# cts198859/deeprl_network

Measured on NVIDIA H100. Metric: agent-env-steps/sec CACC Catch-up NeurComm A2C, higher is better.
Workload: dtype f32

## Files before the change

### deeprl_network_b200/csrc/tc.cuh

```cuda
#pragma once
#include <cuda_runtime.h>
#include <stdint.h>

namespace tc {

__device__ __forceinline__ uint32_t tf32_rn(float x) {
  uint32_t r;
  asm("cvt.rna.tf32.f32 %0, %1;" : "=r"(r) : "f"(x));
  return r;
}
__device__ __forceinline__ void split_tf32(float x, uint32_t& hi, uint32_t& lo) {
  hi = tf32_rn(x);
  lo = tf32_rn(x - __uint_as_float(hi));
}
__device__ __forceinline__ void split_tf32(float x, float& hi, float& lo) {
  uint32_t h, l;
  split_tf32(x, h, l);
  hi = __uint_as_float(h); lo = __uint_as_float(l);
}
__device__ __forceinline__ uint32_t smem_u32(const void* p) { return (uint32_t)__cvta_generic_to_shared(p); }

__device__ __forceinline__ void pdl_wait() { asm volatile("griddepcontrol.wait;" ::: "memory"); }
__device__ __forceinline__ void pdl_launch_dependents() { asm volatile("griddepcontrol.launch_dependents;" ::: "memory"); }

// ... 40 lines not shown
  return false;
}

__device__ __forceinline__ void bulk_g2s(void* smem_dst, const void* gsrc, uint32_t bytes, uint64_t* bar) {
  asm volatile("cp.async.bulk.shared::cluster.global.mbarrier::complete_tx::bytes [%0], [%1], %2, [%3];" ::"r"(
                   smem_u32(smem_dst)),
               "l"(gsrc), "r"(bytes), "r"(smem_u32(bar))
               : "memory");
}

__host__ __device__ inline uint32_t sw128_offset(uint32_t row, uint32_t k) {
  return (row >> 3) * 1024u + (row & 7u) * 128u + ((((k >> 2) ^ row) & 7u) << 4) + ((k & 3u) << 2);
}
__device__ __forceinline__ uint64_t smem_desc_sw128(const void* tile) {
  const uint64_t addr = (uint64_t)(smem_u32(tile) >> 4) & 0x3FFFull;
  return addr | (1ull << 16) | ((uint64_t)(1024 >> 4) << 32) | (1ull << 62);
}
__device__ __forceinline__ void st_hilo8(uint8_t* tile_hi, uint8_t* tile_lo, uint32_t row, uint32_t k0, const float (&x)[8]) {
  float h[8], l[8];
#pragma unroll
  for (int i = 0; i < 8; ++i) split_tf32(x[i], h[i], l[i]);
#pragma unroll
  for (int c = 0; c < 2; ++c) {
    const uint32_t off = sw128_offset(row, k0 + 4 * c);
    *reinterpret_cast<float4*>(tile_hi + off) = make_float4(h[4 * c], h[4 * c + 1], h[4 * c + 2], h[4 * c + 3]);
    *reinterpret_cast<float4*>(tile_lo + off) = make_float4(l[4 * c], l[4 * c + 1], l[4 * c + 2], l[4 * c + 3]);
  }
}
__device__ __forceinline__ void fence_proxy_async() { asm volatile("fence.proxy.async.shared::cta;" ::: "memory"); }

__device__ __forceinline__ void wgmma_fence() { asm volatile("wgmma.fence.sync.aligned;" ::: "memory"); }
__device__ __forceinline__ void wgmma_commit() { asm volatile("wgmma.commit_group.sync.aligned;" ::: "memory"); }
__device__ __forceinline__ void wgmma_wait_all() { asm volatile("wgmma.wait_group.sync.aligned 0;" ::: "memory"); }

__device__ __forceinline__ void wgmma_tf32_n64(float* d, uint64_t da, uint64_t db, uint32_t acc) {
  asm volatile(
      "{\n\t.reg .pred p;\n\tsetp.ne.b32 p, %34, 0;\n\t"
      "wgmma.mma_async.sync.aligned.m64n64k8.f32.tf32.tf32 {%0,%1,%2,%3,%4,%5,%6,%7,%8,%9,%10,%11,%12,%13,%14,%15,%16,%17,%18,%19,%20,%21,%22,%23,%24,%25,%26,%27,%28,%29,%30,%31}, %32, %33, p, 1, 1;\n\t}"
      : "+f"(d[0]), "+f"(d[1]), "+f"(d[2]), "+f"(d[3]), "+f"(d[4]), "+f"(d[5]), "+f"(d[6]), "+f"(d[7]), "+f"(d[8]), "+f"(d[9]), "+f"(d[10]), "+f"(d[11]), "+f"(d[12]), "+f"(d[13]), "+f"(d[14]), "+f"(d[15]), "+f"(d[16]), "+f"(d[17]), "+f"(d[18]), "+f"(d[19]), "+f"(d[20]), "+f"(d[21]), "+f"(d[22]), "+f"(d[23]), "+f"(d[24]), "+f"(d[25]), "+f"(d[26]), "+f"(d[27]), "+f"(d[28]), "+f"(d[29]), "+f"(d[30]), "+f"(d[31])
      : "l"(da), "l"(db), "r"(acc));
}
__device__ __forceinline__ void wgmma_tf32_n128(float* d, uint64_t da, uint64_t db, uint32_t acc) {
  asm volatile(
      "{\n\t.reg .pred p;\n\tsetp.ne.b32 p, %66, 0;\n\t"
      "wgmma.mma_async.sync.aligned.m64n128k8.f32.tf32.tf32 {%0,%1,%2,%3,%4,%5,%6,%7,%8,%9,%10,%11,%12,%13,%14,%15,%16,%17,%18,%19,%20,%21,%22,%23,%24,%25,%26,%27,%28,%29,%30,%31,%32,%33,%34,%35,%36,%37,%38,%39,%40,%41,%42,%43,%44,%45,%46,%47,%48,%49,%50,%51,%52,%53,%54,%55,%56,%57,%58,%59,%60,%61,%62,%63}, %64, %65, p, 1, 1;\n\t}"
      : "+f"(d[0]), "+f"(d[1]), "+f"(d[2]), "+f"(d[3]), "+f"(d[4]), "+f"(d[5]), "+f"(d[6]), "+f"(d[7]), "+f"(d[8]), "+f"(d[9]), "+f"(d[10]), "+f"(d[11]), "+f"(d[12]), "+f"(d[13]), "+f"(d[14]), "+f"(d[15]), "+f"(d[16]), "+f"(d[17]), "+f"(d[18]), "+f"(d[19]), "+f"(d[20]), "+f"(d[21]), "+f"(d[22]), "+f"(d[23]), "+f"(d[24]), "+f"(d[25]), "+f"(d[26]), "+f"(d[27]), "+f"(d[28]), "+f"(d[29]), "+f"(d[30]), "+f"(d[31]), "+f"(d[32]), "+f"(d[33]), "+f"(d[34]), "+f"(d[35]), "+f"(d[36]), "+f"(d[37]), "+f"(d[38]), "+f"(d[39]), "+f"(d[40]), "+f"(d[41]), "+f"(d[42]), "+f"(d[43]), "+f"(d[44]), "+f"(d[45]), "+f"(d[46]), "+f"(d[47]), "+f"(d[48]), "+f"(d[49]), "+f"(d[50]), "+f"(d[51]), "+f"(d[52]), "+f"(d[53]), "+f"(d[54]), "+f"(d[55]), "+f"(d[56]), "+f"(d[57]), "+f"(d[58]), "+f"(d[59]), "+f"(d[60]), "+f"(d[61]), "+f"(d[62]), "+f"(d[63])
      : "l"(da), "l"(db), "r"(acc));
}
__device__ __forceinline__ void wgmma_tf32_n192(float* d, uint64_t da, uint64_t db, uint32_t acc) {
  asm volatile(
      "{\n\t.reg .pred p;\n\tsetp.ne.b32 p, %98, 0;\n\t"
      "wgmma.mma_async.sync.aligned.m64n192k8.f32.tf32.tf32 {%0,%1,%2,%3,%4,%5,%6,%7,%8,%9,%10,%11,%12,%13,%14,%15,%16,%17,%18,%19,%20,%21,%22,%23,%24,%25,%26,%27,%28,%29,%30,%31,%32,%33,%34,%35,%36,%37,%38,%39,%40,%41,%42,%43,%44,%45,%46,%47,%48,%49,%50,%51,%52,%53,%54,%55,%56,%57,%58,%59,%60,%61,%62,%63,%64,%65,%66,%67,%68,%69,%70,%71,%72,%73,%74,%75,%76,%77,%78,%79,%80,%81,%82,%83,%84,%85,%86,%87,%88,%89,%90,%91,%92,%93,%94,%95}, %96, %97, p, 1, 1;\n\t}"
      : "+f"(d[0]), "+f"(d[1]), "+f"(d[2]), "+f"(d[3]), "+f"(d[4]), "+f"(d[5]), "+f"(d[6]), "+f"(d[7]), "+f"(d[8]), "+f"(d[9]), "+f"(d[10]), "+f"(d[11]), "+f"(d[12]), "+f"(d[13]), "+f"(d[14]), "+f"(d[15]), "+f"(d[16]), "+f"(d[17]), "+f"(d[18]), "+f"(d[19]), "+f"(d[20]), "+f"(d[21]), "+f"(d[22]), "+f"(d[23]), "+f"(d[24]), "+f"(d[25]), "+f"(d[26]), "+f"(d[27]), "+f"(d[28]), "+f"(d[29]), "+f"(d[30]), "+f"(d[31]), "+f"(d[32]), "+f"(d[33]), "+f"(d[34]), "+f"(d[35]), "+f"(d[36]), "+f"(d[37]), "+f"(d[38]), "+f"(d[39]), "+f"(d[40]), "+f"(d[41]), "+f"(d[42]), "+f"(d[43]), "+f"(d[44]), "+f"(d[45]), "+f"(d[46]), "+f"(d[47]), "+f"(d[48]), "+f"(d[49]), "+f"(d[50]), "+f"(d[51]), "+f"(d[52]), "+f"(d[53]), "+f"(d[54]), "+f"(d[55]), "+f"(d[56]), "+f"(d[57]), "+f"(d[58]), "+f"(d[59]), "+f"(d[60]), "+f"(d[61]), "+f"(d[62]), "+f"(d[63]), "+f"(d[64]), "+f"(d[65]), "+f"(d[66]), "+f"(d[67]), "+f"(d[68]), "+f"(d[69]), "+f"(d[70]), "+f"(d[71]), "+f"(d[72]), "+f"(d[73]), "+f"(d[74]), "+f"(d[75]), "+f"(d[76]), "+f"(d[77]), "+f"(d[78]), "+f"(d[79]), "+f"(d[80]), "+f"(d[81]), "+f"(d[82]), "+f"(d[83]), "+f"(d[84]), "+f"(d[85]), "+f"(d[86]), "+f"(d[87]), "+f"(d[88]), "+f"(d[89]), "+f"(d[90]), "+f"(d[91]), "+f"(d[92]), "+f"(d[93]), "+f"(d[94]), "+f"(d[95])
      : "l"(da), "l"(db), "r"(acc));
}
__device__ __forceinline__ void wgmma_tf32_n256(float* d, uint64_t da, uint64_t db, uint32_t acc) {
  asm volatile(
      "{\n\t.reg .pred p;\n\tsetp.ne.b32 p, %130, 0;\n\t"
      "wgmma.mma_async.sync.aligned.m64n256k8.f32.tf32.tf32 {%0,%1,%2,%3,%4,%5,%6,%7,%8,%9,%10,%11,%12,%13,%14,%15,%16,%17,%18,%19,%20,%21,%22,%23,%24,%25,%26,%27,%28,%29,%30,%31,%32,%33,%34,%35,%36,%37,%38,%39,%40,%41,%42,%43,%44,%45,%46,%47,%48,%49,%50,%51,%52,%53,%54,%55,%56,%57,%58,%59,%60,%61,%62,%63,%64,%65,%66,%67,%68,%69,%70,%71,%72,%73,%74,%75,%76,%77,%78,%79,%80,%81,%82,%83,%84,%85,%86,%87,%88,%89,%90,%91,%92,%93,%94,%95,%96,%97,%98,%99,%100,%101,%102,%103,%104,%105,%106,%107,%108,%109,%110,%111,%112,%113,%114,%115,%116,%117,%118,%119,%120,%121,%122,%123,%124,%125,%126,%127}, %128, %129, p, 1, 1;\n\t}"
      : "+f"(d[0]), "+f"(d[1]), "+f"(d[2]), "+f"(d[3]), "+f"(d[4]), "+f"(d[5]), "+f"(d[6]), "+f"(d[7]), "+f"(d[8]), "+f"(d[9]), "+f"(d[10]), "+f"(d[11]), "+f"(d[12]), "+f"(d[13]), "+f"(d[14]), "+f"(d[15]), "+f"(d[16]), "+f"(d[17]), "+f"(d[18]), "+f"(d[19]), "+f"(d[20]), "+f"(d[21]), "+f"(d[22]), "+f"(d[23]), "+f"(d[24]), "+f"(d[25]), "+f"(d[26]), "+f"(d[27]), "+f"(d[28]), "+f"(d[29]), "+f"(d[30]), "+f"(d[31]), "+f"(d[32]), "+f"(d[33]), "+f"(d[34]), "+f"(d[35]), "+f"(d[36]), "+f"(d[37]), "+f"(d[38]), "+f"(d[39]), "+f"(d[40]), "+f"(d[41]), "+f"(d[42]), "+f"(d[43]), "+f"(d[44]), "+f"(d[45]), "+f"(d[46]), "+f"(d[47]), "+f"(d[48]), "+f"(d[49]), "+f"(d[50]), "+f"(d[51]), "+f"(d[52]), "+f"(d[53]), "+f"(d[54]), "+f"(d[55]), "+f"(d[56]), "+f"(d[57]), "+f"(d[58]), "+f"(d[59]), "+f"(d[60]), "+f"(d[61]), "+f"(d[62]), "+f"(d[63]), "+f"(d[64]), "+f"(d[65]), "+f"(d[66]), "+f"(d[67]), "+f"(d[68]), "+f"(d[69]), "+f"(d[70]), "+f"(d[71]), "+f"(d[72]), "+f"(d[73]), "+f"(d[74]), "+f"(d[75]), "+f"(d[76]), "+f"(d[77]), "+f"(d[78]), "+f"(d[79]), "+f"(d[80]), "+f"(d[81]), "+f"(d[82]), "+f"(d[83]), "+f"(d[84]), "+f"(d[85]), "+f"(d[86]), "+f"(d[87]), "+f"(d[88]), "+f"(d[89]), "+f"(d[90]), "+f"(d[91]), "+f"(d[92]), "+f"(d[93]), "+f"(d[94]), "+f"(d[95]), "+f"(d[96]), "+f"(d[97]), "+f"(d[98]), "+f"(d[99]), "+f"(d[100]), "+f"(d[101]), "+f"(d[102]), "+f"(d[103]), "+f"(d[104]), "+f"(d[105]), "+f"(d[106]), "+f"(d[107]), "+f"(d[108]), "+f"(d[109]), "+f"(d[110]), "+f"(d[111]), "+f"(d[112]), "+f"(d[113]), "+f"(d[114]), "+f"(d[115]), "+f"(d[116]), "+f"(d[117]), "+f"(d[118]), "+f"(d[119]), "+f"(d[120]), "+f"(d[121]), "+f"(d[122]), "+f"(d[123]), "+f"(d[124]), "+f"(d[125]), "+f"(d[126]), "+f"(d[127])
      : "l"(da), "l"(db), "r"(acc));
}
__device__ __forceinline__ void wgmma_tf32(int N, float* d, uint64_t da, uint64_t db, uint32_t acc) {
  switch (N) {
    case 64: wgmma_tf32_n64(d, da, db, acc); break;
    case 128: wgmma_tf32_n128(d, da, db, acc); break;
    case 192: wgmma_tf32_n192(d, da, db, acc); break;
    default: wgmma_tf32_n256(d, da, db, acc); break;
  }
}
__device__ __forceinline__ void wgmma_kblock_3x(int N, float* d, uint64_t a_hi, uint64_t a_lo, uint64_t b_hi, uint64_t b_lo,
                                                int ksteps, bool first) {
  for (int ks = 0; ks < ksteps; ++ks) {
    wgmma_tf32(N, d, a_hi + 2 * ks, b_hi + 2 * ks, (first && ks == 0) ? 0u : 1u);
    wgmma_tf32(N, d, a_hi + 2 * ks, b_lo + 2 * ks, 1u);
    wgmma_tf32(N, d, a_lo + 2 * ks, b_hi + 2 * ks, 1u);
  }
}

}
```

### deeprl_network_b200/csrc/tc_bwd.cu

```cuda
#include "bwd_common.cuh"
#include "tc_row.cuh"

namespace {
using namespace tcrow;

template <int VAR, bool FM, bool RAW, int HW>
__global__ void __launch_bounds__(TC_THREADS, 1) tc_cell_bwd_kernel(const __grid_constant__ nmarl_model m,
                                                                    const __grid_constant__ BwdK k) {
  extern __shared__ uint8_t smem_raw[];
  const Smem sm = smem_map(smem_raw);
  KbEnt* sched = sm.sched;

  const int i = blockIdx.y;
  const nmarl_agent& ag = m.agent[i];
  const int B = k.B, b0 = blockIdx.x * ROWS;
  const int tid = threadIdx.x, warp = tid >> 5, lane = tid & 31;
  const int n_a = m.n_a, SD = m.s_dim;
  const float* __restrict__ P = k.params;
  constexpr int NGRP = (VAR == NMARL_NC) ? 4 : 2;
  const int Km = (VAR == NMARL_IC3) ? NH : ag.n_nbr * NH;

  if (tid == 0) {
    init_barriers(sm);
    int n = 0;
    const int korder[8] = {4, 5, 0, 1, 6, 7, 2, 3};
    for (int q = 0; q < 8; ++q) sched[n++] = make_kb(ag.tp_gT, SD + NH, NG, korder[q], 0, q == 0, 0, q == 7);
    if (VAR != NMARL_IA2C && Km > 0)
      for (int kb = 0; kb < 2; ++kb) sched[n++] = make_kb(ag.tp_mT, Km, NH, kb, 0, kb == 0, 0, kb == 1);
    *sm.n_kb = n;
  }
  __syncthreads();
  const int n_kb = *sm.n_kb;
  tc::pdl_launch_dependents();
  tc::pdl_wait();

  if (warp < MMA_WARP0) {
    RowCtx c;
    const int set = warp / ROW_WARPS, rh = warp % ROW_WARPS, r = rh * 32 + lane;
    c.a_ring = sm.ast; c.acc = sm.acc; c.r = (uint32_t)r;
    c.a_full = sm.a_full; c.a_empty = sm.a_empty; c.enc_full = sm.enc_full; c.q = 0; c.e = 0; c.set = set; c.err = k.tc_err;
    const int b = b0 + r;
    const size_t row = (size_t)i * B + b;
    const float nd = 1.0f - k.done_pre[b];
    const int e0 = set * EW;
    const float* gates_fm = k.sv_gates + (size_t)i * NG * B;
    const float* sh_fm = k.sv_sh + (size_t)i * (SD + NH) * B;
    const float* enc_fm = k.sv_enc ? k.sv_enc + (size_t)i * 128 * B : nullptr;

    float dh[EW], dct[EW], dzo[EW];
    {
      float dl[HW];
#pragma unroll
      for (int q = 0; q < HW / 4; ++q) {
        const float4 d4 = *reinterpret_cast<const float4*>(k.sv_dlv + row * HW + 4 * q);
        dl[4 * q] = d4.x; dl[4 * q + 1] = d4.y; dl[4 * q + 2] = d4.z; dl[4 * q + 3] = d4.w;
      }
      float dv = 0.f;
#pragma unroll
      for (int cc = 0; cc < HW; ++cc) if (cc == n_a) dv = dl[cc];
      float4 vw[EW / 4];
#pragma unroll
      for (int q4 = 0; q4 < EW / 4; ++q4) vw[q4] = __ldg(reinterpret_cast<const float4*>(P + ag.o_v_w + e0) + q4);
#pragma unroll
      for (int j = 0; j < EW; ++j) {
        float s = 0.f;
// ... 145 lines not shown
#pragma unroll
        for (int j = 0; j < EW; ++j) {
          if (VAR == NMARL_IC3) { o[j] = d[j] * (1.0f - hx[j] * hx[j]); dpm[j] = d[j]; }
          else { o[j] = hx[j] > 0.f ? d[j] : 0.f; dpm[j] = hm[j] > 0.f ? d[j] : 0.f; }
        }
        put_dp(e0, o);
        put_dp(NH + e0, dpm);
      }
    }
    if (VAR != NMARL_IA2C && Km > 0) {
      produce_act(c, dpm);
      tc::mbar_wait(sm.acc_full, 1, k.tc_err, 14);
      const int nblk = (VAR == NMARL_IC3) ? 1 : ag.n_nbr;
      for (int s = 0; s < nblk; ++s) {
        float d[EW];
#pragma unroll
        for (int p = 0; p < EW / 8; ++p) {
          float t[8];
          acc_ld8(c, ACC_COL + s * NH + e0 + 8 * p, t);
#pragma unroll
          for (int j = 0; j < 8; ++j) d[8 * p + j] = t[j];
        }
        if (VAR == NMARL_IC3) {
          const float nn = (float)ag.n_nbr;
#pragma unroll
          for (int j = 0; j < EW; ++j) d[j] /= nn;
          for (int s2 = 0; s2 < ag.n_nbr; ++s2) st_state<FM, EW>(k.dmsg_out, (size_t)i * NMARL_MAX_NBR + s2, b, e0, B, d);
        } else {
          st_state<FM, EW>(k.dmsg_out, (size_t)i * NMARL_MAX_NBR + s, b, e0, B, d);
        }
      }
    }
  } else {
    mma_loop(sched, n_kb, sm.bst, sm.ast, sm.b_full, sm.a_full, sm.a_empty, sm.enc_full, sm.acc_full, sm.acc, k.wpack, k.tc_err);
  }
}

NMARL_PARAMS_FIT(nmarl_model, BwdK);

template <int VAR, bool FM, bool RAW, int HW>
int launch_tc_bwd_fm(const nmarl_model* m, const BwdK& k, cudaStream_t st) {
  auto kern = tc_cell_bwd_kernel<VAR, FM, RAW, HW>;
  static bool configured = false;
  if (!configured) {
    NMARL_CUDA(cudaFuncSetAttribute(kern, cudaFuncAttributeMaxDynamicSharedMemorySize, (int)TC_SMEM));
    configured = true;
  }
  dim3 grid(k.B / ROWS, m->n_agent);
  NMARL_CUDA(nmarl_launch(kern, grid, dim3(TC_THREADS), TC_SMEM, st, true, *m, k));
  NMARL_LAUNCH_CHECK();
  return 0;
}

template <int VAR, int HW>
int launch_tc_bwd_hw(const nmarl_model* m, const BwdK& k, cudaStream_t st) {
  if (k.raw_tiles) return k.state_fm ? launch_tc_bwd_fm<VAR, true, true, HW>(m, k, st) : launch_tc_bwd_fm<VAR, false, true, HW>(m, k, st);
  return k.state_fm ? launch_tc_bwd_fm<VAR, true, false, HW>(m, k, st) : launch_tc_bwd_fm<VAR, false, false, HW>(m, k, st);
}

template <int VAR>
int launch_tc_bwd(const nmarl_model* m, const BwdK& k, cudaStream_t st) {
  return nmarl_head_width(m->n_a) == 8 ? launch_tc_bwd_hw<VAR, 8>(m, k, st) : launch_tc_bwd_hw<VAR, 16>(m, k, st);
}

}

int nmarl_tc_launch_bwd(const nmarl_model* m, const BwdK& k, cudaStream_t st) {
// ... 10 lines not shown
```

### deeprl_network_b200/csrc/tc_cell.cu

```cuda
#include "cell_common.cuh"
#include "tc_row.cuh"

int nmarl_launch_pack_b(const float* W, int ldw, int K, int n0, int nrows, float* out, cudaStream_t st);

namespace {

using namespace tcrow;

template <int VAR, int MODE, bool FM, int HW>
__global__ void __launch_bounds__(TC_THREADS, 1) tc_cell_fwd_kernel(const __grid_constant__ nmarl_model m,
                                                                    const __grid_constant__ FwdK k) {
  constexpr bool SAVE = (MODE == MODE_PS);
  constexpr bool SAMPLE = (MODE == MODE_P || MODE == MODE_PS);
  static_assert(HW <= EW, "a set's HW partial head sums live in its EW gate-f staging columns");
  extern __shared__ uint8_t smem_raw[];
  const Smem sm = smem_map(smem_raw);
  KbEnt* sched = sm.sched;

  const nmarl_fwd_args& a = k.a;
  const int i = blockIdx.y;
  const nmarl_agent& ag = m.agent[i];
  const int B = a.B, b0 = blockIdx.x * ROWS;
  const int tid = threadIdx.x, warp = tid >> 5, lane = tid & 31;
  const int n_a = m.n_a, SD = m.s_dim;
  const float* __restrict__ P = a.params;
  const int Kx = ag.x_nsrc * ag.x_w;

  if (tid == 0) {
    init_barriers(sm);
    int n = 0;
    const int KG = SD + NH, nG = KG / 32;
    sched[n++] = make_kb(ag.tp_x, 64, Kx, 0, ACC_COL, 1, 0, 0);
    if (VAR == NMARL_NC && ag.n_nbr > 0) sched[n++] = make_kb(ag.tp_p, 64, ag.n_nbr * n_a, 0, ACC_COL + 64, 1, 0, 0);
    if (VAR != NMARL_IA2C) {
      const int nM = (VAR == NMARL_IC3) ? 2 : 2 * ag.n_nbr;
      const int KM = (VAR == NMARL_IC3) ? NH : NH * ag.n_nbr;
      const int mcol = (VAR == NMARL_NC) ? ACC_COL + 128 : ACC_COL + 64;
      for (int j = 0; j < nM; ++j) sched[n++] = make_kb(ag.tp_m, 64, KM, j, mcol, j == 0, 0, 0);
    }
    sched[n - 1].last_enc = 1;
    for (int g = 0; g < nG; ++g) sched[n++] = make_kb(ag.tp_g, 256, KG, g, ACC_COL, g == 0, 0, g == nG - 1);
    if (VAR == NMARL_DIAL && MODE != MODE_V)
      for (int j = 0; j < 2; ++j) sched[n++] = make_kb(ag.tp_mfc, 64, NH, j, ACC_COL, j == 0, j == 1, 0);
    *sm.n_kb = n;
  }
  __syncthreads();
  const int n_kb = *sm.n_kb;
  tc::pdl_launch_dependents();
  tc::pdl_wait();

  if (warp < MMA_WARP0) {
    RowCtx c;
    const int set = warp / ROW_WARPS, rh = warp % ROW_WARPS, r = rh * 32 + lane;
    c.a_ring = sm.ast; c.acc = sm.acc; c.r = (uint32_t)r;
    c.a_full = sm.a_full; c.a_empty = sm.a_empty; c.enc_full = sm.enc_full; c.q = 0; c.e = 0; c.set = set; c.err = a.tc_err;
    const int b = b0 + r;
    const size_t row = (size_t)i * B + b;
    const float nd = 1.0f - a.done[b];
    const int LDI = m.kx_pad + m.kp_pad + m.km_pad;
    float* xin_fm = SAVE ? a.sv_xin + (size_t)i * LDI * B : nullptr;
    float* sh_fm = SAVE ? a.sv_sh + (size_t)i * (SD + NH) * B : nullptr;
    float* enc_fm = (SAVE && a.sv_enc) ? a.sv_enc + (size_t)i * 128 * B : nullptr;
    float* gates_fm = SAVE ? a.sv_gates + (size_t)i * NG * B : nullptr;
    long long* prof = (k.prof != nullptr && blockIdx.x == 0 && blockIdx.y == 1 && tid == 0) ? k.prof : nullptr;
    int pi_ = 0;
#define STAMP() do { if (prof) prof[pi_++] = clock64(); } while (0)
    STAMP();
    const int c0 = set * W;
    const int e0 = set * EW;

    const int inv_xw = 65536 / ag.x_w + 1, inv_na = 65536 / n_a + 1;
    float xv[W];
#pragma unroll
    for (int j = 0; j < W; ++j) {
      const int kk = c0 + j;
      float val = 0.f;
      if (kk < Kx) {
        const int s = (kk * inv_xw) >> 16, f = kk - s * ag.x_w;
        val = a.obs[((size_t)ag.x_src[s] * B + b) * m.obs_stride + f];
      }
// ... 173 lines not shown
          gf[x] = r1 * di;
          go[x] = r2 * du;
          gu[x] = fmaf(2.0f, r2 * dO, -1.0f);
          cn[x] = gf[x] * (cpv[x] * nd) + gi[x] * gu[x];
        }
      }
#pragma unroll
      for (int x = 0; x < 8; x += 2) {
        const float d0 = 1.0f + __expf(fminf(-2.0f * cn[x], 40.0f)), d1 = 1.0f + __expf(fminf(-2.0f * cn[x + 1], 40.0f));
        const float r = frcp_(d0 * d1);
        hn[x] = go[x] * fmaf(2.0f, r * d1, -1.0f);
        hn[x + 1] = go[x + 1] * fmaf(2.0f, r * d0, -1.0f);
      }
      STAMP();
      if (MODE != MODE_V) {
        st_state<FM, 8>(a.c_out, (size_t)i, b, u0, B, cn);
        st_state<FM, 8>(a.h_out, (size_t)i, b, u0, B, hn);
      }
      if (SAVE) {
        st_fm<8>(gates_fm, 0 * NH + u0, B, b, gi); st_fm<8>(gates_fm, 1 * NH + u0, B, b, gf);
        st_fm<8>(gates_fm, 2 * NH + u0, B, b, go); st_fm<8>(gates_fm, 3 * NH + u0, B, b, gu);
      }
      STAMP();
      if (MODE != MODE_V) {
        if (n_a == 4) {
#pragma unroll
          for (int x = 0; x < 8; ++x) {
            const float4 w4 = __ldg(reinterpret_cast<const float4*>(P + ag.o_pi_w) + u0 + x);
            logit[0] = fmaf(hn[x], w4.x, logit[0]); logit[1] = fmaf(hn[x], w4.y, logit[1]);
            logit[2] = fmaf(hn[x], w4.z, logit[2]); logit[3] = fmaf(hn[x], w4.w, logit[3]);
          }
        } else {
#pragma unroll
          for (int x = 0; x < 8; ++x)
#pragma unroll
            for (int cc = 0; cc < HW; ++cc)
              if (cc < n_a) logit[cc] = fmaf(hn[x], __ldg(P + ag.o_pi_w + (u0 + x) * n_a + cc), logit[cc]);
        }
      }
      if (!SAMPLE) {
        const float4 v0 = __ldg(reinterpret_cast<const float4*>(P + ag.o_v_w + u0)), v1 = __ldg(reinterpret_cast<const float4*>(P + ag.o_v_w + u0) + 1);
        v = fmaf(hn[0], v0.x, v); v = fmaf(hn[1], v0.y, v); v = fmaf(hn[2], v0.z, v); v = fmaf(hn[3], v0.w, v);
        v = fmaf(hn[4], v1.x, v); v = fmaf(hn[5], v1.y, v); v = fmaf(hn[6], v1.z, v); v = fmaf(hn[7], v1.w, v);
      }
      STAMP();
      if (VAR == NMARL_DIAL && MODE != MODE_V) {
#pragma unroll
        for (int x = 0; x < 8; ++x) s0[(u0 - e0) + x] = hn[x];
      }
    }
    if (VAR == NMARL_DIAL && MODE != MODE_V) produce_act(c, s0);

    {
      float* hp = sm.acc;
#pragma unroll
      for (int cc = 0; cc < HW - 1; ++cc) hp[acc_idx(r, NH + e0 + cc)] = logit[cc];
      hp[acc_idx(r, NH + e0 + HW - 1)] = v;
    }
    STAMP();
    row_barrier();
    STAMP();
    if (set == 0) {
#pragma unroll
      for (int cc = 0; cc < HW; ++cc) logit[cc] = 0.f;
      v = 0.f;
#pragma unroll
      for (int s = 0; s < NSET; ++s) {
        const float* hp = sm.acc;
#pragma unroll
// ... 26 lines not shown
          else u = philox_u01(a.rng[0], a.rng[1] + a.rng_offset, (uint32_t)row, 0x41435431u);
          double cdf[HW];
          double s = 0.0;
#pragma unroll
          for (int cc = 0; cc < HW; ++cc) { if (cc < n_a) s += (double)pi[cc]; cdf[cc] = s; }
          if (a.sample_mode == NMARL_SAMPLE_UNIFORM) {
#pragma unroll
            for (int cc = 0; cc < HW; ++cc) if (cc < n_a) act += ((cdf[cc] / s) <= u) ? 1 : 0;
          } else {
            const double us = u * s;
#pragma unroll
            for (int cc = 0; cc < HW; ++cc) if (cc < n_a) act += (cdf[cc] <= us) ? 1 : 0;
          }
          act = min(act, n_a - 1);
        }
        a.action[row] = act;
      }
      if (!SAMPLE) {
        for (int s = 0; s < ag.n_nbr; ++s) v += __ldg(P + ag.o_v_w + NH + s * n_a + a.act_in[(size_t)ag.nbr[s] * B + b]);
        v += __ldg(P + ag.o_v_b);
        if (a.v != nullptr) a.v[row] = v;
      }
    }
    if (VAR == NMARL_DIAL && MODE != MODE_V) {
      float mo[EW];
      enc_wait(c);
      enc_load(c, ACC_COL, mo);
      bias_act(mo, P + ag.o_mfc_b + e0, 0);
      st_state<FM, EW>(a.msg_out, (size_t)i, b, e0, B, mo);
    }
    STAMP();
    if (prof) prof[31] = pi_;
  } else {
    mma_loop(sched, n_kb, sm.bst, sm.ast, sm.b_full, sm.a_full, sm.a_empty, sm.enc_full, sm.acc_full, sm.acc, a.wpack, a.tc_err);
  }
  __syncthreads();
}


NMARL_PARAMS_FIT(nmarl_model, FwdK);

template <int VAR, int MODE, bool FM, int HW>
int launch_tc_fm(const nmarl_model* m, const FwdK& k, cudaStream_t st) {
  auto kern = tc_cell_fwd_kernel<VAR, MODE, FM, HW>;
  static bool configured = false;
  if (!configured) {
    NMARL_CUDA(cudaFuncSetAttribute(kern, cudaFuncAttributeMaxDynamicSharedMemorySize, (int)TC_SMEM));
    configured = true;
  }
  dim3 grid(k.a.B / ROWS, m->n_agent);
  FwdK k2 = k;
  k2.prof = g_nmarl_prof;
  NMARL_CUDA(nmarl_launch(kern, grid, dim3(TC_THREADS), TC_SMEM, st, true, *m, k2));
  NMARL_LAUNCH_CHECK();
  return 0;
}

template <int VAR, int MODE, int HW>
int launch_tc_hw(const nmarl_model* m, const FwdK& k, cudaStream_t st) {
  return k.a.state_fm ? launch_tc_fm<VAR, MODE, true, HW>(m, k, st) : launch_tc_fm<VAR, MODE, false, HW>(m, k, st);
}

template <int VAR, int MODE>
int launch_tc(const nmarl_model* m, const FwdK& k, cudaStream_t st) {
  return nmarl_head_width(m->n_a) == 8 ? launch_tc_hw<VAR, MODE, 8>(m, k, st) : launch_tc_hw<VAR, MODE, 16>(m, k, st);
}

// ... 87 lines not shown
```

### deeprl_network_b200/csrc/tc_row.cuh

```cuda
#pragma once
#include "common.cuh"
#include "tc.cuh"

namespace tcrow {

constexpr int ROWS = 64;
constexpr int S_STAGES = 2;
constexpr uint32_t STAGE_BYTES = 2 * 256 * 128;
constexpr int A_SLOTS = 2;
constexpr uint32_t A_TILE = ROWS * 128, A_SLOT_BYTES = 2 * A_TILE;
static_assert((A_SLOTS & (A_SLOTS - 1)) == 0, "A ring slots: power of two");
constexpr int ACC_COLS = 256;
constexpr uint32_t ACC_BYTES = ROWS * ACC_COLS * 4;
constexpr uint32_t ACC_COL = 0;
constexpr int MAX_KB = 24;
constexpr int NSET = 4;
constexpr int W = 32 / NSET, EW = 64 / NSET;
constexpr int ROW_WARPS = ROWS / 32;
constexpr int ROW_THREADS = ROWS * NSET;
constexpr int MMA_WARP0 = ROW_THREADS / 32;
constexpr int TC_THREADS = ROW_THREADS + 128;
static_assert(MMA_WARP0 % 4 == 0, "the MMA warps must form an aligned warpgroup");
static_assert(W == 8 && EW % 8 == 0, "8-column operand pieces");

__device__ __forceinline__ uint32_t acc_idx(uint32_t row, uint32_t col) {
  return row * ACC_COLS + (col & ~31u) + ((((col >> 2) ^ row) & 7u) << 2) + (col & 3u);
}

struct KbEnt {
  uint32_t off_bytes, bytes;
  uint16_t dcol;
  uint8_t ksteps, first, last_enc, last_acc, pad0, pad1;
};

struct RowCtx {
  uint8_t* a_ring; const float* acc;
  uint32_t r;
  uint64_t* a_full; uint64_t* a_empty; uint64_t* enc_full;
  int q, e, set;
  int* err;
};

__device__ __forceinline__ void produce_begin(RowCtx& c) {
  const int slot = c.q & (A_SLOTS - 1);
  tc::mbar_wait(&c.a_empty[slot], ((c.q / A_SLOTS) & 1) ^ 1, c.err, 11);
}
__device__ __forceinline__ void produce_piece(RowCtx& c, int col , const float (&x)[8]) {
  uint8_t* hi = c.a_ring + (c.q & (A_SLOTS - 1)) * A_SLOT_BYTES;
  tc::st_hilo8(hi, hi + A_TILE, c.r, (uint32_t)col, x);
}
__device__ __forceinline__ void produce_end(RowCtx& c) {
  tc::fence_proxy_async();
  tc::mbar_arrive(&c.a_full[c.q & (A_SLOTS - 1)]);
  c.q++;
}
__device__ __forceinline__ void acc_ld8(const RowCtx& c, uint32_t col, float (&v)[8]) {
#pragma unroll
  for (int h = 0; h < 2; ++h) {
    const float4 t = *reinterpret_cast<const float4*>(c.acc + acc_idx(c.r, col + 4 * h));
    v[4 * h] = t.x; v[4 * h + 1] = t.y; v[4 * h + 2] = t.z; v[4 * h + 3] = t.w;
  }
}
__device__ __forceinline__ void produce_in(RowCtx& c, const float (&x)[W]) {
  produce_begin(c);
  produce_piece(c, c.set * W, x);
// ... 62 lines not shown
#pragma unroll
    for (int j = 0; j < NV; ++j) p[(size_t)j * B] = v[j];
  } else {
    float* p = base + (plane * (size_t)B + b) * NH + u0;
#pragma unroll
    for (int q = 0; q < NV / 4; ++q) *reinterpret_cast<float4*>(p + 4 * q) = make_float4(v[4 * q], v[4 * q + 1], v[4 * q + 2], v[4 * q + 3]);
  }
}
template <int NV>
__device__ __forceinline__ void store_vec(float* dst, const float (&s)[NV]) {
#pragma unroll
  for (int q = 0; q < NV / 4; ++q) *reinterpret_cast<float4*>(dst + 4 * q) = make_float4(s[4 * q], s[4 * q + 1], s[4 * q + 2], s[4 * q + 3]);
}
__device__ __forceinline__ void bias_act(float (&v)[EW], const float* __restrict__ b, int act ) {
#pragma unroll
  for (int q = 0; q < EW / 4; ++q) {
    const float4 bb = __ldg(reinterpret_cast<const float4*>(b) + q);
    const float z[4] = {v[4 * q] + bb.x, v[4 * q + 1] + bb.y, v[4 * q + 2] + bb.z, v[4 * q + 3] + bb.w};
#pragma unroll
    for (int j = 0; j < 4; ++j) v[4 * q + j] = act == 0 ? fmaxf(z[j], 0.f) : (act == 1 ? tanhf(z[j]) : z[j]);
  }
}
__device__ __forceinline__ float frcp_(float x) {
  float r;
  asm("rcp.approx.ftz.f32 %0, %1;" : "=f"(r) : "f"(x));
  return r;
}
__device__ __forceinline__ float fsigmoid(float x) { return frcp_(1.0f + __expf(-x)); }
__device__ __forceinline__ float ftanh(float x) { return fmaf(2.0f, frcp_(1.0f + __expf(-2.0f * x)), -1.0f); }
__device__ __forceinline__ void row_barrier() { asm volatile("bar.sync 1, %0;" ::"n"(ROW_THREADS) : "memory"); }
__device__ __forceinline__ void mma_wg_sync() { asm volatile("bar.sync 2, 128;" ::: "memory"); }


__device__ __forceinline__ void mma_loop(const KbEnt* sched, int n_kb, uint8_t* bst, uint8_t* ast, uint64_t* b_full,
                                         uint64_t* a_full, uint64_t* a_empty, uint64_t* enc_full, uint64_t* acc_full,
                                         float* acc_s, const float* wpack, int* err) {
  const int t = threadIdx.x - MMA_WARP0 * 32, w = t >> 5, l = t & 31;
  const uint8_t* wp = reinterpret_cast<const uint8_t*>(wpack);
  auto fetch = [&](int q) {
    const int st = q % S_STAGES;
    const KbEnt e = sched[q];
    tc::mbar_arrive_expect_tx(&b_full[st], e.bytes);
    tc::bulk_g2s(bst + st * STAGE_BYTES, wp + e.off_bytes, e.bytes, &b_full[st]);
  };
  if (t == 0)
    for (int q = 0; q < S_STAGES && q < n_kb; ++q) fetch(q);
  float d[128];
#pragma unroll
  for (int j = 0; j < 128; ++j) d[j] = 0.f;
  for (int q = 0; q < n_kb; ++q) {
    const int st = q % S_STAGES, slot = q & (A_SLOTS - 1);
    const KbEnt e = sched[q];
    tc::mbar_wait(&b_full[st], (q / S_STAGES) & 1, err, 31);
    tc::mbar_wait(&a_full[slot], (q / A_SLOTS) & 1, err, 32);
    const int N = (int)(e.bytes / 256);
    uint8_t* b = bst + st * STAGE_BYTES;
    uint8_t* a = ast + slot * A_SLOT_BYTES;
    tc::wgmma_fence();
    tc::wgmma_kblock_3x(N, d, tc::smem_desc_sw128(a), tc::smem_desc_sw128(a + A_TILE), tc::smem_desc_sw128(b),
                        tc::smem_desc_sw128(b + N * 128), e.ksteps, e.first != 0);
    tc::wgmma_commit();
    tc::wgmma_wait_all();
    tc::mbar_arrive(&a_empty[slot]);
    mma_wg_sync();
    if (t == 0 && q + S_STAGES < n_kb) fetch(q + S_STAGES);
    if (e.last_enc || e.last_acc || q + 1 == n_kb || sched[q + 1].first) {
      const uint32_t r0 = 16 * w + (l >> 2);
#pragma unroll
      for (int j = 0; j < 32; ++j) {
        if (8 * j < N) {
          const uint32_t col = e.dcol + 8 * j + 2 * (l & 3);
#pragma unroll
          for (int h = 0; h < 2; ++h) {
            const uint32_t r = r0 + 8 * h;
            *reinterpret_cast<float2*>(acc_s + acc_idx(r, col)) = make_float2(d[4 * j + 2 * h], d[4 * j + 2 * h + 1]);
          }
        }
      }
      if (e.last_enc) tc::mbar_arrive(enc_full);
      if (e.last_acc) tc::mbar_arrive(acc_full);
    }
  }
}
__device__ __forceinline__ KbEnt make_kb(int off_floats, int N, int K, int kb, int dcol, int first, int last_enc, int last_acc) {
  KbEnt e;
  e.off_bytes = (uint32_t)(off_floats + kb * 2 * N * 32) * 4u;
  e.bytes = 2u * N * 128u;
  const int k8 = (K + 7) / 8 * 8;
  e.ksteps = (uint8_t)min(4, (k8 - kb * 32) / 8);
  e.dcol = (uint16_t)dcol; e.first = first; e.last_enc = last_enc; e.last_acc = last_acc;
  e.pad0 = e.pad1 = 0;
  return e;
}
struct Smem {
  uint8_t* bst; uint8_t* ast; float* acc;
  uint64_t *b_full, *a_full, *a_empty, *enc_full, *acc_full;
  int* n_kb; KbEnt* sched;
};
__device__ __forceinline__ Smem smem_map(uint8_t* raw) {
  uint8_t* s = reinterpret_cast<uint8_t*>((reinterpret_cast<uintptr_t>(raw) + 1023) & ~uintptr_t(1023));
  Smem m;
  m.bst = s;
  m.ast = s + S_STAGES * STAGE_BYTES;
  m.acc = reinterpret_cast<float*>(m.ast + A_SLOTS * A_SLOT_BYTES);
  uint64_t* bars = reinterpret_cast<uint64_t*>(reinterpret_cast<uint8_t*>(m.acc) + ACC_BYTES);
  m.b_full = bars; m.a_full = bars + S_STAGES; m.a_empty = m.a_full + A_SLOTS;
  m.enc_full = m.a_empty + A_SLOTS; m.acc_full = m.enc_full + 1;
  m.n_kb = reinterpret_cast<int*>(m.acc_full + 1);
  m.sched = reinterpret_cast<KbEnt*>(m.n_kb + 2);
  return m;
}
__device__ __forceinline__ void init_barriers(const Smem& s) {
  for (int i = 0; i < S_STAGES; ++i) tc::mbar_init(&s.b_full[i], 1);
  for (int i = 0; i < A_SLOTS; ++i) { tc::mbar_init(&s.a_full[i], ROW_THREADS); tc::mbar_init(&s.a_empty[i], 128); }
  tc::mbar_init(s.enc_full, 128);
  tc::mbar_init(s.acc_full, 128);
  tc::fence_barrier_init();
}
constexpr size_t TC_SMEM = 1024  + S_STAGES * STAGE_BYTES + A_SLOTS * A_SLOT_BYTES + ACC_BYTES + 16 * 8  +
                           8 + MAX_KB * sizeof(KbEnt);
static_assert(TC_SMEM <= 232448, "cell kernels exceed the 227 KB of dynamic shared memory");

}
```

Before: 46.03 million.

## Specialize wgmma loop per segment width and pipeline k-blocks with wait_group 1

Replaces the flat per-k-block schedule with segments whose N width and final k-step count are compile-time template parameters. Each segment keeps an accumulator array sized to its width, and in the cell kernel successive k-blocks overlap by waiting on only the previous wgmma group. The runtime switch on N and the full wait after every k-block go away, at the cost of more template instantiations and code size. It also reorders the policy-logit loop nest.

```diff
diff --git a/deeprl_network_b200/csrc/tc.cuh b/deeprl_network_b200/csrc/tc.cuh
--- a/deeprl_network_b200/csrc/tc.cuh
+++ b/deeprl_network_b200/csrc/tc.cuh
@@ -96,6 +96,8 @@
 __device__ __forceinline__ void wgmma_fence() { asm volatile("wgmma.fence.sync.aligned;" ::: "memory"); }
 __device__ __forceinline__ void wgmma_commit() { asm volatile("wgmma.commit_group.sync.aligned;" ::: "memory"); }
 __device__ __forceinline__ void wgmma_wait_all() { asm volatile("wgmma.wait_group.sync.aligned 0;" ::: "memory"); }
+template <int N>
+__device__ __forceinline__ void wgmma_wait() { asm volatile("wgmma.wait_group.sync.aligned %0;" ::"n"(N) : "memory"); }
 
 __device__ __forceinline__ void wgmma_tf32_n64(float* d, uint64_t da, uint64_t db, uint32_t acc) {
   asm volatile(
@@ -133,6 +135,23 @@
     default: wgmma_tf32_n256(d, da, db, acc); break;
   }
 }
+template <int N>
+__device__ __forceinline__ void wgmma_tf32(float* d, uint64_t da, uint64_t db, uint32_t acc) {
+  static_assert(N == 64 || N == 128 || N == 192 || N == 256, "wgmma tf32 widths used here");
+  if constexpr (N == 64) wgmma_tf32_n64(d, da, db, acc);
+  else if constexpr (N == 128) wgmma_tf32_n128(d, da, db, acc);
+  else if constexpr (N == 192) wgmma_tf32_n192(d, da, db, acc);
+  else wgmma_tf32_n256(d, da, db, acc);
+}
+template <int N, int KS>
+__device__ __forceinline__ void wgmma_kblock_3x(float* d, uint64_t a_hi, uint64_t a_lo, uint64_t b_hi, uint64_t b_lo, bool first) {
+#pragma unroll
+  for (int ks = 0; ks < KS; ++ks) {
+    wgmma_tf32<N>(d, a_hi + 2 * ks, b_hi + 2 * ks, (first && ks == 0) ? 0u : 1u);
+    wgmma_tf32<N>(d, a_hi + 2 * ks, b_lo + 2 * ks, 1u);
+    wgmma_tf32<N>(d, a_lo + 2 * ks, b_hi + 2 * ks, 1u);
+  }
+}
 __device__ __forceinline__ void wgmma_kblock_3x(int N, float* d, uint64_t a_hi, uint64_t a_lo, uint64_t b_hi, uint64_t b_lo,
                                                 int ksteps, bool first) {
   for (int ks = 0; ks < ksteps; ++ks) {
diff --git a/deeprl_network_b200/csrc/tc_bwd.cu b/deeprl_network_b200/csrc/tc_bwd.cu
--- a/deeprl_network_b200/csrc/tc_bwd.cu
+++ b/deeprl_network_b200/csrc/tc_bwd.cu
@@ -9,7 +9,6 @@
                                                                     const __grid_constant__ BwdK k) {
   extern __shared__ uint8_t smem_raw[];
   const Smem sm = smem_map(smem_raw);
-  KbEnt* sched = sm.sched;
 
   const int i = blockIdx.y;
   const nmarl_agent& ag = m.agent[i];
@@ -22,15 +21,13 @@
 
   if (tid == 0) {
     init_barriers(sm);
-    int n = 0;
+    SchedBuilder sb(sm);
     const int korder[8] = {4, 5, 0, 1, 6, 7, 2, 3};
-    for (int q = 0; q < 8; ++q) sched[n++] = make_kb(ag.tp_gT, SD + NH, NG, korder[q], 0, q == 0, 0, q == 7);
-    if (VAR != NMARL_IA2C && Km > 0)
-      for (int kb = 0; kb < 2; ++kb) sched[n++] = make_kb(ag.tp_mT, Km, NH, kb, 0, kb == 0, 0, kb == 1);
-    *sm.n_kb = n;
+    sb.gemm(ag.tp_gT, SD + NH, NG, 0, DONE_ACC, korder);
+    if (VAR != NMARL_IA2C && Km > 0) sb.gemm(ag.tp_mT, Km, NH, 0, DONE_ACC);
+    sb.finish();
   }
   __syncthreads();
-  const int n_kb = *sm.n_kb;
   tc::pdl_launch_dependents();
   tc::pdl_wait();
 
@@ -242,7 +239,7 @@
       }
     }
   } else {
-    mma_loop(sched, n_kb, sm.bst, sm.ast, sm.b_full, sm.a_full, sm.a_empty, sm.enc_full, sm.acc_full, sm.acc, k.wpack, k.tc_err);
+    mma_loop<0, 64, 128, 192, 256>(sm, k.wpack, k.tc_err);
   }
 }
 
diff --git a/deeprl_network_b200/csrc/tc_cell.cu b/deeprl_network_b200/csrc/tc_cell.cu
--- a/deeprl_network_b200/csrc/tc_cell.cu
+++ b/deeprl_network_b200/csrc/tc_cell.cu
@@ -15,7 +15,6 @@
   static_assert(HW <= EW, "a set's HW partial head sums live in its EW gate-f staging columns");
   extern __shared__ uint8_t smem_raw[];
   const Smem sm = smem_map(smem_raw);
-  KbEnt* sched = sm.sched;
 
   const nmarl_fwd_args& a = k.a;
   const int i = blockIdx.y;
@@ -28,24 +27,19 @@
 
   if (tid == 0) {
     init_barriers(sm);
-    int n = 0;
-    const int KG = SD + NH, nG = KG / 32;
-    sched[n++] = make_kb(ag.tp_x, 64, Kx, 0, ACC_COL, 1, 0, 0);
-    if (VAR == NMARL_NC && ag.n_nbr > 0) sched[n++] = make_kb(ag.tp_p, 64, ag.n_nbr * n_a, 0, ACC_COL + 64, 1, 0, 0);
+    SchedBuilder sb(sm);
+    sb.gemm(ag.tp_x, 64, Kx, ACC_COL, DONE_NONE);
+    if (VAR == NMARL_NC) sb.gemm(ag.tp_p, 64, ag.n_nbr * n_a, ACC_COL + 64, DONE_NONE);
     if (VAR != NMARL_IA2C) {
-      const int nM = (VAR == NMARL_IC3) ? 2 : 2 * ag.n_nbr;
       const int KM = (VAR == NMARL_IC3) ? NH : NH * ag.n_nbr;
-      const int mcol = (VAR == NMARL_NC) ? ACC_COL + 128 : ACC_COL + 64;
-      for (int j = 0; j < nM; ++j) sched[n++] = make_kb(ag.tp_m, 64, KM, j, mcol, j == 0, 0, 0);
-    }
-    sched[n - 1].last_enc = 1;
-    for (int g = 0; g < nG; ++g) sched[n++] = make_kb(ag.tp_g, 256, KG, g, ACC_COL, g == 0, 0, g == nG - 1);
-    if (VAR == NMARL_DIAL && MODE != MODE_V)
-      for (int j = 0; j < 2; ++j) sched[n++] = make_kb(ag.tp_mfc, 64, NH, j, ACC_COL, j == 0, j == 1, 0);
-    *sm.n_kb = n;
+      sb.gemm(ag.tp_m, 64, KM, (VAR == NMARL_NC) ? ACC_COL + 128 : ACC_COL + 64, DONE_NONE);
+    }
+    sm.seg[sb.ns - 1].done = DONE_ENC;
+    sb.gemm(ag.tp_g, 256, SD + NH, ACC_COL, DONE_ACC);
+    if (VAR == NMARL_DIAL && MODE != MODE_V) sb.gemm(ag.tp_mfc, 64, NH, ACC_COL, DONE_ENC);
+    sb.finish();
   }
   __syncthreads();
-  const int n_kb = *sm.n_kb;
   tc::pdl_launch_dependents();
   tc::pdl_wait();
 
@@ -285,9 +279,9 @@
           }
         } else {
 #pragma unroll
-          for (int x = 0; x < 8; ++x)
-#pragma unroll
-            for (int cc = 0; cc < HW; ++cc)
+          for (int cc = 0; cc < HW; ++cc)
+#pragma unroll
+            for (int x = 0; x < 8; ++x)
               if (cc < n_a) logit[cc] = fmaf(hn[x], __ldg(P + ag.o_pi_w + (u0 + x) * n_a + cc), logit[cc]);
         }
       }
@@ -380,7 +374,7 @@
     STAMP();
     if (prof) prof[31] = pi_;
   } else {
-    mma_loop(sched, n_kb, sm.bst, sm.ast, sm.b_full, sm.a_full, sm.a_empty, sm.enc_full, sm.acc_full, sm.acc, a.wpack, a.tc_err);
+    mma_loop<MMA_PIPE | MMA_PARTIAL, 64, 256>(sm, a.wpack, a.tc_err);
   }
   __syncthreads();
 }
diff --git a/deeprl_network_b200/csrc/tc_row.cuh b/deeprl_network_b200/csrc/tc_row.cuh
--- a/deeprl_network_b200/csrc/tc_row.cuh
+++ b/deeprl_network_b200/csrc/tc_row.cuh
@@ -27,10 +27,12 @@
   return row * ACC_COLS + (col & ~31u) + ((((col >> 2) ^ row) & 7u) << 2) + (col & 3u);
 }
 
-struct KbEnt {
-  uint32_t off_bytes, bytes;
-  uint16_t dcol;
-  uint8_t ksteps, first, last_enc, last_acc, pad0, pad1;
+constexpr int MAX_SEG = 8;
+struct KbEnt { uint32_t off_bytes, bytes; };
+enum : uint8_t { DONE_NONE = 0, DONE_ENC, DONE_ACC };
+struct Seg {
+  uint16_t n, dcol;
+  uint8_t kb0, nkb, ks_last, done;
 };
 
 struct RowCtx {
@@ -159,71 +161,117 @@
 __device__ __forceinline__ void mma_wg_sync() { asm volatile("bar.sync 2, 128;" ::: "memory"); }
 
 
-__device__ __forceinline__ void mma_loop(const KbEnt* sched, int n_kb, uint8_t* bst, uint8_t* ast, uint64_t* b_full,
-                                         uint64_t* a_full, uint64_t* a_empty, uint64_t* enc_full, uint64_t* acc_full,
-                                         float* acc_s, const float* wpack, int* err) {
-  const int t = threadIdx.x - MMA_WARP0 * 32, w = t >> 5, l = t & 31;
-  const uint8_t* wp = reinterpret_cast<const uint8_t*>(wpack);
-  auto fetch = [&](int q) {
-    const int st = q % S_STAGES;
-    const KbEnt e = sched[q];
-    tc::mbar_arrive_expect_tx(&b_full[st], e.bytes);
-    tc::bulk_g2s(bst + st * STAGE_BYTES, wp + e.off_bytes, e.bytes, &b_full[st]);
-  };
-  if (t == 0)
-    for (int q = 0; q < S_STAGES && q < n_kb; ++q) fetch(q);
-  float d[128];
-#pragma unroll
-  for (int j = 0; j < 128; ++j) d[j] = 0.f;
-  for (int q = 0; q < n_kb; ++q) {
-    const int st = q % S_STAGES, slot = q & (A_SLOTS - 1);
-    const KbEnt e = sched[q];
-    tc::mbar_wait(&b_full[st], (q / S_STAGES) & 1, err, 31);
-    tc::mbar_wait(&a_full[slot], (q / A_SLOTS) & 1, err, 32);
-    const int N = (int)(e.bytes / 256);
-    uint8_t* b = bst + st * STAGE_BYTES;
-    uint8_t* a = ast + slot * A_SLOT_BYTES;
-    tc::wgmma_fence();
-    tc::wgmma_kblock_3x(N, d, tc::smem_desc_sw128(a), tc::smem_desc_sw128(a + A_TILE), tc::smem_desc_sw128(b),
-                        tc::smem_desc_sw128(b + N * 128), e.ksteps, e.first != 0);
-    tc::wgmma_commit();
-    tc::wgmma_wait_all();
-    tc::mbar_arrive(&a_empty[slot]);
-    mma_wg_sync();
-    if (t == 0 && q + S_STAGES < n_kb) fetch(q + S_STAGES);
-    if (e.last_enc || e.last_acc || q + 1 == n_kb || sched[q + 1].first) {
-      const uint32_t r0 = 16 * w + (l >> 2);
-#pragma unroll
-      for (int j = 0; j < 32; ++j) {
-        if (8 * j < N) {
-          const uint32_t col = e.dcol + 8 * j + 2 * (l & 3);
-#pragma unroll
-          for (int h = 0; h < 2; ++h) {
-            const uint32_t r = r0 + 8 * h;
-            *reinterpret_cast<float2*>(acc_s + acc_idx(r, col)) = make_float2(d[4 * j + 2 * h], d[4 * j + 2 * h + 1]);
-          }
-        }
-      }
-      if (e.last_enc) tc::mbar_arrive(enc_full);
-      if (e.last_acc) tc::mbar_arrive(acc_full);
-    }
-  }
-}
-__device__ __forceinline__ KbEnt make_kb(int off_floats, int N, int K, int kb, int dcol, int first, int last_enc, int last_acc) {
-  KbEnt e;
-  e.off_bytes = (uint32_t)(off_floats + kb * 2 * N * 32) * 4u;
-  e.bytes = 2u * N * 128u;
-  const int k8 = (K + 7) / 8 * 8;
-  e.ksteps = (uint8_t)min(4, (k8 - kb * 32) / 8);
-  e.dcol = (uint16_t)dcol; e.first = first; e.last_enc = last_enc; e.last_acc = last_acc;
-  e.pad0 = e.pad1 = 0;
-  return e;
-}
 struct Smem {
   uint8_t* bst; uint8_t* ast; float* acc;
   uint64_t *b_full, *a_full, *a_empty, *enc_full, *acc_full;
-  int* n_kb; KbEnt* sched;
-};
+  int* n_kb; int* n_seg; KbEnt* sched; Seg* seg;
+};
+
+struct SchedBuilder {
+  const Smem& s;
+  int nk, ns;
+  __device__ __forceinline__ explicit SchedBuilder(const Smem& sm) : s(sm), nk(0), ns(0) {}
+  __device__ __forceinline__ void gemm(int off_floats, int N, int K, int dcol, uint8_t done, const int* order = nullptr) {
+    const int nkb = (K + 31) / 32;
+    if (nkb == 0) return;
+    int kb = 0;
+    for (int j = 0; j < nkb; ++j) {
+      kb = order ? order[j] : j;
+      s.sched[nk + j] = KbEnt{(uint32_t)(off_floats + kb * 2 * N * 32) * 4u, 2u * N * 128u};
+    }
+    const int k8 = (K + 7) / 8 * 8;
+    s.seg[ns++] = Seg{(uint16_t)N, (uint16_t)dcol, (uint8_t)nk, (uint8_t)nkb, (uint8_t)min(4, (k8 - kb * 32) / 8), done};
+    nk += nkb;
+  }
+  __device__ __forceinline__ void finish() { *s.n_kb = nk; *s.n_seg = ns; }
+};
+
+struct MmaCtx {
+  const Smem& s;
+  const uint8_t* wp;
+  int* err;
+  int t, n_kb;
+  __device__ __forceinline__ void fetch(int q) const {
+    const int st = q % S_STAGES;
+    const KbEnt e = s.sched[q];
+    tc::mbar_arrive_expect_tx(&s.b_full[st], e.bytes);
+    tc::bulk_g2s(s.bst + st * STAGE_BYTES, wp + e.off_bytes, e.bytes, &s.b_full[st]);
+  }
+  __device__ __forceinline__ void release(int q) const {
+    tc::mbar_arrive(&s.a_empty[q & (A_SLOTS - 1)]);
+    mma_wg_sync();
+    if (t == 0 && q + S_STAGES < n_kb) fetch(q + S_STAGES);
+  }
+  template <int N, int KS>
+  __device__ __forceinline__ void issue(float* d, int q, bool first) const {
+    const int st = q % S_STAGES, slot = q & (A_SLOTS - 1);
+    tc::mbar_wait(&s.b_full[st], (q / S_STAGES) & 1, err, 31);
+    tc::mbar_wait(&s.a_full[slot], (q / A_SLOTS) & 1, err, 32);
+    const uint8_t* b = s.bst + st * STAGE_BYTES;
+    const uint8_t* a = s.ast + slot * A_SLOT_BYTES;
+    tc::wgmma_fence();
+    tc::wgmma_kblock_3x<N, KS>(d, tc::smem_desc_sw128(a), tc::smem_desc_sw128(a + A_TILE), tc::smem_desc_sw128(b),
+                               tc::smem_desc_sw128(b + N * 128), first);
+    tc::wgmma_commit();
+  }
+};
+
+enum : int { MMA_PIPE = 1, MMA_PARTIAL = 2 };
+
+template <int OPT, int N, int KS_LAST>
+__device__ __forceinline__ void gemm_segment(const MmaCtx& x, const Seg& sg) {
+  float d[N / 2];
+#pragma unroll
+  for (int j = 0; j < N / 2; ++j) d[j] = 0.f;
+  const int q0 = sg.kb0, qe = q0 + sg.nkb - 1;
+  constexpr bool PIPE = (OPT & MMA_PIPE) != 0;
+  for (int q = q0; q < qe; ++q) {
+    x.issue<N, 4>(d, q, q == q0);
+    if (!PIPE) { tc::wgmma_wait<0>(); x.release(q); }
+    else if (q > q0) { tc::wgmma_wait<1>(); x.release(q - 1); }
+  }
+  x.issue<N, KS_LAST>(d, qe, qe == q0);
+  tc::wgmma_wait<0>();
+  if (PIPE && qe > q0) x.release(qe - 1);
+  x.release(qe);
+  const int w = x.t >> 5, l = x.t & 31;
+  const uint32_t r0 = 16 * w + (l >> 2);
+#pragma unroll
+  for (int j = 0; j < N / 8; ++j) {
+    const uint32_t col = sg.dcol + 8 * j + 2 * (l & 3);
+#pragma unroll
+    for (int h = 0; h < 2; ++h)
+      *reinterpret_cast<float2*>(x.s.acc + acc_idx(r0 + 8 * h, col)) = make_float2(d[4 * j + 2 * h], d[4 * j + 2 * h + 1]);
+  }
+}
+template <int OPT, int N>
+__device__ __forceinline__ bool gemm_segment_n(const MmaCtx& x, const Seg& sg) {
+  if (sg.n != N) return false;
+  if constexpr (N == 64 && (OPT & MMA_PARTIAL) != 0) {
+    switch (sg.ks_last) {
+      case 1: gemm_segment<OPT, N, 1>(x, sg); return true;
+      case 2: gemm_segment<OPT, N, 2>(x, sg); return true;
+      case 3: gemm_segment<OPT, N, 3>(x, sg); return true;
+    }
+  }
+  if (sg.ks_last != 4) return false;
+  gemm_segment<OPT, N, 4>(x, sg);
+  return true;
+}
+template <int OPT, int... NS>
+__device__ __forceinline__ void mma_loop(const Smem& s, const float* wpack, int* err) {
+  const MmaCtx x{s, reinterpret_cast<const uint8_t*>(wpack), err, (int)threadIdx.x - MMA_WARP0 * 32, *s.n_kb};
+  if (x.t == 0)
+    for (int q = 0; q < S_STAGES && q < x.n_kb; ++q) x.fetch(q);
+  const int n_seg = *s.n_seg;
+  for (int i = 0; i < n_seg; ++i) {
+    const Seg sg = s.seg[i];
+    const bool known = (gemm_segment_n<OPT, NS>(x, sg) || ...);
+    if (!known) { if (x.t == 0) atomicCAS(err, 0, 30); break; }
+    if (sg.done == DONE_ENC) tc::mbar_arrive(s.enc_full);
+    if (sg.done == DONE_ACC) tc::mbar_arrive(s.acc_full);
+  }
+}
 __device__ __forceinline__ Smem smem_map(uint8_t* raw) {
   uint8_t* s = reinterpret_cast<uint8_t*>((reinterpret_cast<uintptr_t>(raw) + 1023) & ~uintptr_t(1023));
   Smem m;
@@ -234,7 +282,9 @@
   m.b_full = bars; m.a_full = bars + S_STAGES; m.a_empty = m.a_full + A_SLOTS;
   m.enc_full = m.a_empty + A_SLOTS; m.acc_full = m.enc_full + 1;
   m.n_kb = reinterpret_cast<int*>(m.acc_full + 1);
+  m.n_seg = m.n_kb + 1;
   m.sched = reinterpret_cast<KbEnt*>(m.n_kb + 2);
+  m.seg = reinterpret_cast<Seg*>(m.sched + MAX_KB);
   return m;
 }
 __device__ __forceinline__ void init_barriers(const Smem& s) {
@@ -245,7 +295,7 @@
   tc::fence_barrier_init();
 }
 constexpr size_t TC_SMEM = 1024  + S_STAGES * STAGE_BYTES + A_SLOTS * A_SLOT_BYTES + ACC_BYTES + 16 * 8  +
-                           8 + MAX_KB * sizeof(KbEnt);
+                           8 + MAX_KB * sizeof(KbEnt) + MAX_SEG * sizeof(Seg);
 static_assert(TC_SMEM <= 232448, "cell kernels exceed the 227 KB of dynamic shared memory");
 
 }
```

Result: faster. 53.08 million (median of 6 runs) (+15.3%).
